# Picsart-AI-Research/StreamingT2V

Hardware: NVIDIA H100
Metric: denoise_steps_per_sec (higher is better)
Workload: dtype bf16

## Files before the change

streamingt2v_b200/csrc/mtgemm.cu:

```cuda
#include <cuda.h>
#include <cuda_bf16.h>
#include <stdlib.h>
#include <string.h>

#include "../../include/b200svd.h"
#include "common.h"
#include "mtgemm_ring.h"
#include "ptx.cuh"
#include "wgmma.cuh"

namespace b200 {

struct GemmDev {
  int32_t tap_off[B200SVD_MAX_TAPS][5];
  uint32_t taps, kblocks;
  uint32_t n;
  uint32_t n_tiles;
  uint32_t total_tiles;
  uint32_t m_ext[3];
  uint32_t m_lb[3];
  uint32_t m_tiles[3];
  uint32_t m_adim[3];
  int64_t out_rs[3];
  void* out;
  int64_t ldo;
  int32_t out_fp32;
  const float* bias;
  const float* fvec;
  int64_t ldf;
  uint32_t rows_per_frame;
  int32_t act;
  float s_acc;
  const __nv_bfloat16* res1;
  int64_t ld1;
  float s1;
  const __nv_bfloat16* res2;
  int64_t ld2;
  float s2;
  float* gn_part;
  int32_t* gn_slot_sample;
  int64_t gn_ld;
  uint32_t gn_rows;
  int32_t staged;
  int32_t epi_kind;
  uint32_t stages;
  uint32_t res_slots;
  uint32_t wg_off[3];
  const float* slope;
#ifdef MTGEMM_PHASE_CLOCKS
  long long* phase_buf;
// ... 69 lines not shown
  static constexpr int PRODUCER_REGS = 40;
  static constexpr int RES_SLOTS_AT_MIN = (SMEM_LIMIT - FIXED_BYTES - MIN_STAGES * STAGE_BYTES) / RES_SLOT_BYTES;
  static int res_slots_fit(int stages) { return (SMEM_LIMIT - FIXED_BYTES - stages * STAGE_BYTES) / RES_SLOT_BYTES; }
  static_assert(STAGES >= 4, "pipeline depth without residuals");
  static_assert(RES_SLOTS_AT_MIN >= 2, "two residuals need two ring slots");
  static_assert(STAGES * STAGE_BYTES + FIXED_BYTES <= SMEM_LIMIT, "shared memory budget");
  static_assert(STAGE_BYTES % 1024 == 0, "stage alignment");
  static_assert(BN % SUB_W == 0, "sub-tiles");
};

constexpr int ALT_STG_SLOT_BYTES = BM * SUB_W * 2;
constexpr int ALT_STG_BYTES = 2 * STG_SLOTS * ALT_STG_SLOT_BYTES;
template <int BN>
struct AltCfg {
  static constexpr int B_STAGE_BYTES = BN * BK * 2;
  static constexpr int STAGE_BYTES = A_STAGE_BYTES + B_STAGE_BYTES;
  static constexpr int FIXED = ALT_STG_BYTES + BAR_BYTES;
  static constexpr int STAGES_FIT = (SMEM_LIMIT - FIXED) / STAGE_BYTES;
  static constexpr int STAGES = STAGES_FIT > MAX_STAGES ? MAX_STAGES : STAGES_FIT;
  static constexpr int SUBTILES = BN / SUB_W;
  static constexpr int CONSUMER_REGS = 232;
  static constexpr int PRODUCER_REGS = 40;
  static constexpr int RES_SLOTS_AT_MIN = (SMEM_LIMIT - FIXED - MIN_STAGES * STAGE_BYTES) / RES_SLOT_BYTES;
  static int res_slots_fit(int stages) { return (SMEM_LIMIT - FIXED - stages * STAGE_BYTES) / RES_SLOT_BYTES; }
  static_assert(BN <= 128, "128 x BN accumulator in one warpgroup's registers");
  static_assert(2 * 128 * CONSUMER_REGS + 128 * PRODUCER_REGS <= 65536, "register file");
  static_assert(STAGES >= 4, "pipeline depth without residuals");
  static_assert(RES_SLOTS_AT_MIN >= 2, "two residuals need two ring slots");
  static_assert(STAGES * STAGE_BYTES + FIXED <= SMEM_LIMIT, "shared memory budget");
  static_assert(STAGE_BYTES % 1024 == 0, "stage alignment");
  static_assert(BN % SUB_W == 0, "sub-tiles");
};

__device__ __forceinline__ void decode_tile(const GemmDev& p, uint32_t tile, uint32_t& n_tile, uint32_t& mb1,
                                            uint32_t& mb2, uint32_t& mb3) {
  n_tile = tile % p.n_tiles;
  uint32_t mt = tile / p.n_tiles;
  const uint32_t t1 = mt % p.m_tiles[0];
  mt /= p.m_tiles[0];
  const uint32_t t2 = mt % p.m_tiles[1];
  const uint32_t t3 = mt / p.m_tiles[1];
  mb1 = t1 << p.m_lb[0];
  mb2 = t2 << p.m_lb[1];
  mb3 = t3 << p.m_lb[2];
}

__device__ __forceinline__ float ldg_bf16(const __nv_bfloat16* p) { return __bfloat162float(p[0]); }

__device__ __forceinline__ void load_bf16_pair(const __nv_bfloat16* base, int64_t i, bool both, float& a, float& b) {
  if (both && (i & 1) == 0) {
    const uint32_t w = __ldg(reinterpret_cast<const unsigned int*>(base + i));
    a = bf16_lo(w);
    b = bf16_hi(w);
  } else {
    a = ldg_bf16(base + i);
    b = both ? ldg_bf16(base + i + 1) : 0.f;
  }
}

__device__ __forceinline__ float epi_act(int act, float s_acc, float v, float g) {
  if (act == B200SVD_ACT_SILU) {
    v = silu_fast(v);
  } else if (act == B200SVD_ACT_GELU) {
    v = gelu_fast(v);
  } else if (act == B200SVD_ACT_GEGLU) {
    v = __fmul_rn(v, gelu_fast(g));
  } else if (act == B200SVD_ACT_PRELU) {
    v = v > 0.f ? v : __fmul_rn(g, v);
  }
  return __fmul_rn(v, s_acc);
// ... 162 lines not shown
#pragma unroll
    for (int o = 4; o < 32; o <<= 1) {
      gs0 += __shfl_xor_sync(0xffffffffu, gs0, o);
      gs1 += __shfl_xor_sync(0xffffffffu, gs1, o);
      gq0 += __shfl_xor_sync(0xffffffffu, gq0, o);
      gq1 += __shfl_xor_sync(0xffffffffu, gq1, o);
    }
    if (sender && first_row) *reinterpret_cast<float4*>(gxb + 2 * (8 * jj + 2 * cq)) = make_float4(gs0, gq0, gs1, gq1);
    if (!sender) {
      acc[4 * j] = gs0;
      acc[4 * j + 1] = gq0;
      acc[4 * j + 2] = gs1;
      acc[4 * j + 3] = gq1;
    }
  }
}

__device__ __forceinline__ void gn_write_partials(const GemmDev& p, const EpiTile& t, const float* acc, int c,
                                                  uint32_t cq, const float* gxb, uint32_t slot) {
  float2* dst = reinterpret_cast<float2*>(p.gn_part) + (int64_t)slot * p.gn_ld;
#pragma unroll
  for (int jj = 0; jj < 4; ++jj) {
    const int j = 4 * c + jj;
    const uint32_t ocol = t.otile0 + (uint32_t)(8 * j) + 2 * cq;
    if (ocol < t.n_out) {
      const float4 o = *reinterpret_cast<const float4*>(gxb + 2 * (8 * jj + 2 * cq));
      dst[ocol] = make_float2(acc[4 * j] + o.x, acc[4 * j + 1] + o.y);
      if (ocol + 1 < t.n_out) dst[ocol + 1] = make_float2(acc[4 * j + 2] + o.z, acc[4 * j + 3] + o.w);
    }
  }
}

template <int BN>
__device__ __forceinline__ void produce_ab(const GemmDev& p, const CUtensorMap* tmA, const CUtensorMap* tmB,
                                           uint8_t* smem, uint64_t* full_bar, uint64_t* empty_bar) {
  constexpr int STAGE_BYTES = A_STAGE_BYTES + BN * BK * 2;
  PhaseClock pc;
  uint32_t st = 0, ph = 0;
  for (uint32_t tile = blockIdx.x; tile < p.total_tiles; tile += gridDim.x) {
    uint32_t n_tile, mb1, mb2, mb3;
    decode_tile(p, tile, n_tile, mb1, mb2, mb3);
    int base[5] = {0, 0, 0, 0, 0};
    base[p.m_adim[0]] += (int)mb1;
    base[p.m_adim[1]] += (int)mb2;
    base[p.m_adim[2]] += (int)mb3;
    const int n0 = (int)(n_tile * BN);
    for (uint32_t tap = 0; tap < p.taps; ++tap) {
      const int c0 = p.tap_off[tap][0];
      const int c1 = base[1] + p.tap_off[tap][1];
      const int c2 = base[2] + p.tap_off[tap][2];
      const int c3 = base[3] + p.tap_off[tap][3];
      const int c4 = base[4] + p.tap_off[tap][4];
#pragma unroll 1
      for (uint32_t kb = 0; kb < p.kblocks; ++kb) {
        pc.mark(PC_OTHER);
        mbar_wait_parked(&empty_bar[st], ph ^ 1);
        pc.mark(PC_RING_WAIT);
        uint8_t* sa = smem + st * STAGE_BYTES;
        mbar_expect_tx(&full_bar[st], STAGE_BYTES);
        tma_load_5d(sa, tmA, &full_bar[st], c0 + (int)(kb * BK), c1, c2, c3, c4);
        tma_load_3d(sa + A_STAGE_BYTES, tmB, &full_bar[st], (int)(kb * BK), n0, (int)tap);
        if (++st == p.stages) {
          st = 0;
          ph ^= 1;
        }
      }
    }
  }
  pc.write(PC_BUF(p), 0);
}

__device__ __forceinline__ void produce_residuals(const GemmDev& p, const CUtensorMap* tmR1, const CUtensorMap* tmR2,
                                                  uint8_t* res_smem, uint64_t* res_full, uint64_t* res_empty,
                                                  uint32_t tile_out_w, uint32_t n_out) {
  if (p.res1 != nullptr) prefetch_tmap(tmR1);
  if (p.res2 != nullptr) prefetch_tmap(tmR2);
  uint32_t slot = 0, ph = 0;
  for (uint32_t tile = blockIdx.x; tile < p.total_tiles; tile += gridDim.x) {
    uint32_t n_tile, mb1, mb2, mb3;
    decode_tile(p, tile, n_tile, mb1, mb2, mb3);
    const uint32_t otile0 = n_tile * tile_out_w;
    for (uint32_t c = 0; c < tile_out_w / SUB_W && otile0 + c * SUB_W < n_out; ++c) {
      for (int r = 0; r < 2; ++r) {
        if ((r == 0 ? p.res1 : p.res2) == nullptr) continue;
        mbar_wait_parked(&res_empty[slot], ph ^ 1);
        mbar_expect_tx(&res_full[slot], RES_SLOT_BYTES);
        tma_load_4d(res_smem + slot * RES_SLOT_BYTES, r == 0 ? tmR1 : tmR2, &res_full[slot],
                    (int)(otile0 + c * SUB_W), (int)mb1, (int)mb2, (int)mb3);
        if (++slot == p.res_slots) {
          slot = 0;
          ph ^= 1;
        }
      }
    }
  }
}

template <int BN, class E, int HALVES>
__device__ __forceinline__ void epilogue_staged(const GemmDev& p, const CUtensorMap* tmO, const EpiTile& t,
                                                float* const (&acc)[HALVES], const OutRow (&rows)[HALVES][2],
                                                uint8_t* stg_smem, const uint8_t* res_smem, uint64_t* res_full,
                                                uint64_t* res_empty, RingPos& rr, uint32_t& stg_it, uint32_t cw,
                                                uint32_t rbase, uint32_t cq, bool leader, float* gn_x, PhaseClock& pc) {
  constexpr uint32_t SLOT_BYTES = HALVES * STG_SLOT_BYTES;
  const uint8_t* res_rows = res_smem + (HALVES == 1 ? cw * STG_SLOT_BYTES : 0u);
  const uint32_t wl = rbase >> 4, rq = rbase & 7u;
#pragma unroll
  for (int c = 0; c < BN / SUB_W; ++c) {
    if (E::geglu(p) && c >= BN / SUB_W / 2) break;
    if (t.otile0 + (uint32_t)(c * SUB_W) >= t.n_out) break;
    uint8_t* stg = stg_smem + (cw * STG_SLOTS + (stg_it & 1)) * SLOT_BYTES;
    float bv[4][2], gbv[4][2];
    epi_load_bias<BN, E>(p, t, c, cq, bv, gbv);
    const uint8_t* r1s = res_rows;
    const uint8_t* r2s = res_rows;
    uint32_t r1slot = 0, r2slot = 0;
    pc.mark(PC_EPI);
    if (E::res1(p)) {
      r1slot = rr.idx;
      mbar_wait(&res_full[rr.idx], rr.phase);
      r1s = res_rows + rr.idx * RES_SLOT_BYTES;
      ring_step(rr, p.res_slots);
    }
    if (E::res2(p)) {
      r2slot = rr.idx;
      mbar_wait(&res_full[rr.idx], rr.phase);
      r2s = res_rows + rr.idx * RES_SLOT_BYTES;
      ring_step(rr, p.res_slots);
// ... 2 lines not shown
#pragma unroll
    for (int hh = 0; hh < HALVES; ++hh)
      epi_stage_half<BN, E>(p, t, acc[hh], c, rbase, cq, stg + hh * STG_SLOT_BYTES, r1s + hh * STG_SLOT_BYTES,
                            r2s + hh * STG_SLOT_BYTES, bv, gbv, rows[hh]);
    float* gxb = nullptr;
    if constexpr (HALVES == 1 && E::GENERIC) {
      gxb = gn_x + ((cw * 2 + (stg_it & 1)) * 2 + (wl >> 1)) * (SUB_W * 2);
      if (p.gn_part != nullptr) gn_sum_partials<BN>(t, acc[0], c, rbase, cq, stg, rows[0], gxb, wl & 1, rq == 0);
    }
    fence_proxy_async_smem();
    pc.mark(PC_EPI);
    if (leader) tma_store_wait_read0();
    named_bar_sync(5 + (int)cw, 128);
    pc.mark(PC_STORE_WAIT);
    if (leader) {
      if (E::res1(p)) mbar_arrive(&res_empty[r1slot]);
      if (E::res2(p)) mbar_arrive(&res_empty[r2slot]);
      const bool second = HALVES == 1 && cw != 0;
      tma_store_4d(tmO, stg, (int)(t.otile0 + c * SUB_W), (int)(t.mb1 + (second ? p.wg_off[0] : 0u)),
                   (int)(t.mb2 + (second ? p.wg_off[1] : 0u)), (int)(t.mb3 + (second ? p.wg_off[2] : 0u)));
      tma_store_commit();
    }
    if constexpr (HALVES == 1 && E::GENERIC) {
      if (p.gn_part != nullptr && (wl & 1) == 0 && rq == 0)
        gn_write_partials(p, t, acc[0], c, cq, gxb, t.mt * 4u + 2 * cw + (wl >> 1));
    }
    ++stg_it;
  }
}

template <int BN>
__global__ void __launch_bounds__(NUM_THREADS, 1)
mtgemm_kernel(const __grid_constant__ CUtensorMap tmA, const __grid_constant__ CUtensorMap tmB,
              const __grid_constant__ CUtensorMap tmO, const __grid_constant__ CUtensorMap tmR1,
              const __grid_constant__ CUtensorMap tmR2, const GemmDev p) {
  using Cfg = TileCfg<BN>;
  constexpr int R = BN / 2;
  extern __shared__ __align__(1024) uint8_t smem[];
  if ((smem_u32(smem) & 1023u) != 0) __trap();
  const uint32_t stages = p.stages, rslots = p.res_slots;
  uint8_t* res_smem = smem + stages * Cfg::STAGE_BYTES;
  uint8_t* stg_smem = res_smem + rslots * RES_SLOT_BYTES;
  float* gn_x = reinterpret_cast<float*>(stg_smem + STG_BYTES);
  uint64_t* full_bar = reinterpret_cast<uint64_t*>(stg_smem + STG_BYTES + GN_BYTES);
  uint64_t* empty_bar = full_bar + MAX_STAGES;
  uint64_t* res_full = empty_bar + MAX_STAGES;
  uint64_t* res_empty = res_full + MAX_RES_SLOTS;

  const int warp = threadIdx.x >> 5;
  const int lane = threadIdx.x & 31;
  const int wg = warp >> 2;
  const uint32_t iters_per_tile = p.taps * p.kblocks;
  const bool geglu = (p.act == B200SVD_ACT_GEGLU);
  const uint32_t n_out = geglu ? p.n / 2 : p.n;
  const uint32_t tile_out_w = geglu ? (uint32_t)BN / 2 : (uint32_t)BN;

  if (threadIdx.x == 0) {
    prefetch_tmap(&tmA);
    prefetch_tmap(&tmB);
    if (p.staged) prefetch_tmap(&tmO);
    for (uint32_t s = 0; s < stages; ++s) {
      mbar_init(&full_bar[s], 1);
      mbar_init(&empty_bar[s], 2);
    }
    for (uint32_t s = 0; s < rslots; ++s) {
      mbar_init(&res_full[s], 1);
      mbar_init(&res_empty[s], 2);
    }
    fence_barrier_init();
  }
  __syncthreads();

  if (wg == 0) {
    asm volatile("setmaxnreg.dec.sync.aligned.u32 %0;" ::"n"(Cfg::PRODUCER_REGS));
    if (threadIdx.x == 0) {
      produce_ab<BN>(p, &tmA, &tmB, smem, full_bar, empty_bar);
    } else if (threadIdx.x == 32 && rslots != 0) {
      produce_residuals(p, &tmR1, &tmR2, res_smem, res_full, res_empty, tile_out_w, n_out);
    }
    return;
  }
  asm volatile("setmaxnreg.inc.sync.aligned.u32 %0;" ::"n"(Cfg::CONSUMER_REGS));

  const int cw = wg - 1;
  const int wl = warp & 3;
  const int rq = lane >> 2, cq = lane & 3;
  const bool leader = (threadIdx.x & 127) == 0;
  const uint32_t rbase = (uint32_t)(16 * wl + rq);
  RingPos ab = {0, 0};
  RingPos rr = {0, 0};
  uint32_t stg_it = 0;
  float acc[R];
  PhaseClock pc;

  for (uint32_t tile = blockIdx.x; tile < p.total_tiles; tile += gridDim.x) {
    pc.mark(PC_EPI);
#pragma unroll
    for (int i = 0; i < R; ++i) acc[i] = 0.f;
    uint32_t prev = 0;
    for (uint32_t i = 0; i < iters_per_tile; ++i) {
      mbar_wait(&full_bar[ab.idx], ab.phase);
      pc.mark(PC_RING_WAIT);
      const uint32_t sa = smem_u32(smem + ab.idx * Cfg::STAGE_BYTES);
      const uint64_t adesc = smem_desc_k_sw128(sa + cw * (A_STAGE_BYTES / 2));
      const uint64_t bdesc = smem_desc_k_sw128(sa + A_STAGE_BYTES);
      wgmma_fence_regs(acc);
      wgmma_fence();
#pragma unroll
      for (int kk = 0; kk < BK / 16; ++kk)
        Wgmma<BN>::ss(acc, adesc + (uint64_t)(kk * 2), bdesc + (uint64_t)(kk * 2), 1u);
      wgmma_commit();
      wgmma_fence_regs(acc);
      wgmma_wait<1>();
      pc.mark(PC_MMA);
      if (i > 0 && leader) mbar_arrive(&empty_bar[prev]);
      prev = ab.idx;
      ring_step(ab, stages);
    }
    wgmma_wait<0>();
    pc.mark(PC_MMA);
    wgmma_fence_regs(acc);
    if (leader) mbar_arrive(&empty_bar[prev]);

    uint32_t n_tile, mb1, mb2, mb3;
    decode_tile(p, tile, n_tile, mb1, mb2, mb3);
    const EpiTile et = {n_tile * BN, n_tile * tile_out_w, n_out, mb1, mb2, mb3, tile / p.n_tiles};
    const OutRow rows[1][2] = {{out_row(p, et, 64 * cw + rbase), out_row(p, et, 64 * cw + rbase + 8)}};
    if (p.staged) {
      float* const accs[1] = {acc};
      switch (p.epi_kind) {
        case B200SVD_EPI_GENERIC:
          epilogue_staged<BN, EpiGeneric, 1>(p, &tmO, et, accs, rows, stg_smem, res_smem, res_full, res_empty, rr,
                                             stg_it, cw, rbase, cq, leader, gn_x, pc);
          break;
#define MTGEMM_CASE(ID, ACT, BIAS, FVEC, NRES)                                                                    \
  case ID:                                                                                                        \
    if constexpr (ACT != B200SVD_ACT_GEGLU || BN == 128 || BN == 256)                                             \
      epilogue_staged<BN, Epi<ACT, BIAS, FVEC, NRES>, 1>(p, &tmO, et, accs, rows, stg_smem, res_smem, res_full,   \
                                                         res_empty, rr, stg_it, cw, rbase, cq, leader, gn_x, pc); \
    break;
        MTGEMM_EPI_KINDS(MTGEMM_CASE)
#undef MTGEMM_CASE
      }
      if (p.gn_part != nullptr && (wl & 1) == 0 && lane == 0 && n_tile == 0) {
        const uint32_t slot = et.mt * 4u + (uint32_t)(2 * cw + (wl >> 1));
        p.gn_slot_sample[slot] = rows[0][0].valid ? (int32_t)((uint32_t)rows[0][0].row / p.gn_rows) : -1;
      }
      continue;
    }
    constexpr int NJ = BN / 8;
#pragma unroll
    for (int j = 0; j < NJ; ++j) {
      if (geglu && j >= NJ / 2) break;
      const uint32_t tcol = 8 * j + 2 * cq;
      const uint32_t ocol = et.otile0 + tcol;
      const bool in0 = ocol < n_out, in1 = ocol + 1 < n_out;
#pragma unroll
      for (int h = 0; h < 2; ++h) {
        float v0 = acc[4 * j + 2 * h], v1 = acc[4 * j + 2 * h + 1];
// ... 25 lines not shown
          float a, b;
          load_bf16_pair(p.res1, row * p.ld1 + ocol, in1, a, b);
          v0 = __fmaf_rn(p.s1, a, v0);
          v1 = __fmaf_rn(p.s1, b, v1);
        }
        if (p.res2 != nullptr) {
          float a, b;
          load_bf16_pair(p.res2, row * p.ld2 + ocol, in1, a, b);
          v0 = __fmaf_rn(p.s2, a, v0);
          v1 = __fmaf_rn(p.s2, b, v1);
        }
        if (p.out_fp32) {
          float* op = reinterpret_cast<float*>(p.out) + row * p.ldo + ocol;
          if (in1 && ((row * p.ldo + ocol) & 1) == 0) {
            *reinterpret_cast<float2*>(op) = make_float2(v0, v1);
          } else {
            op[0] = v0;
            if (in1) op[1] = v1;
          }
        } else {
          __nv_bfloat16* op = reinterpret_cast<__nv_bfloat16*>(p.out) + row * p.ldo + ocol;
          if (in1) {
            *reinterpret_cast<uint32_t*>(op) = pack_bf16x2(v0, v1);
          } else {
            op[0] = __float2bfloat16(v0);
          }
        }
      }
    }
  }
  pc.mark(PC_EPI);
  if (leader) pc.write(PC_BUF(p), 1 + cw);
  if (p.staged && leader) tma_store_wait_all();
}

template <int BN>
__global__ void __launch_bounds__(NUM_THREADS, 1)
mtgemm_alt_kernel(const __grid_constant__ CUtensorMap tmA, const __grid_constant__ CUtensorMap tmB,
                  const __grid_constant__ CUtensorMap tmO, const __grid_constant__ CUtensorMap tmR1,
                  const __grid_constant__ CUtensorMap tmR2, const GemmDev p) {
  using Cfg = AltCfg<BN>;
  constexpr int R = BN / 2;
  extern __shared__ __align__(1024) uint8_t smem[];
  if ((smem_u32(smem) & 1023u) != 0) __trap();
  const uint32_t stages = p.stages, rslots = p.res_slots;
  uint8_t* res_smem = smem + stages * Cfg::STAGE_BYTES;
  uint8_t* stg_smem = res_smem + rslots * RES_SLOT_BYTES;
  uint64_t* full_bar = reinterpret_cast<uint64_t*>(stg_smem + ALT_STG_BYTES);
  uint64_t* empty_bar = full_bar + MAX_STAGES;
  uint64_t* res_full = empty_bar + MAX_STAGES;
  uint64_t* res_empty = res_full + MAX_RES_SLOTS;
  uint32_t* tiles_done = reinterpret_cast<uint32_t*>(res_empty + MAX_RES_SLOTS);

  const int warp = threadIdx.x >> 5;
  const int lane = threadIdx.x & 31;
  const int wg = warp >> 2;
  const uint32_t iters_per_tile = p.taps * p.kblocks;
  const bool geglu = (p.act == B200SVD_ACT_GEGLU);
  const uint32_t n_out = geglu ? p.n / 2 : p.n;
  const uint32_t tile_out_w = geglu ? (uint32_t)BN / 2 : (uint32_t)BN;

  if (threadIdx.x == 0) {
    prefetch_tmap(&tmA);
    prefetch_tmap(&tmB);
    prefetch_tmap(&tmO);
    for (int i = 0; i < 4; ++i) tiles_done[i] = 0;
    for (uint32_t s = 0; s < stages; ++s) {
      mbar_init(&full_bar[s], 1);
      mbar_init(&empty_bar[s], 1);
    }
    for (uint32_t s = 0; s < rslots; ++s) {
      mbar_init(&res_full[s], 1);
      mbar_init(&res_empty[s], 1);
    }
    fence_barrier_init();
  }
  __syncthreads();

  if (wg == 0) {
    asm volatile("setmaxnreg.dec.sync.aligned.u32 %0;" ::"n"(Cfg::PRODUCER_REGS));
    if (threadIdx.x == 0) {
      produce_ab<BN>(p, &tmA, &tmB, smem, full_bar, empty_bar);
    } else if (threadIdx.x == 32 && rslots != 0) {
      produce_residuals(p, &tmR1, &tmR2, res_smem, res_full, res_empty, tile_out_w, n_out);
    }
    return;
  }
  asm volatile("setmaxnreg.inc.sync.aligned.u32 %0;" ::"n"(Cfg::CONSUMER_REGS));

  const uint32_t cw = (uint32_t)(wg - 1);
  const int wl = warp & 3;
  const int rq = lane >> 2, cq = lane & 3;
  const bool leader = (threadIdx.x & 127) == 0;
  const uint32_t rbase = (uint32_t)(16 * wl + rq);
  const uint32_t nres = (p.res1 != nullptr ? 1u : 0u) + (p.res2 != nullptr ? 1u : 0u);
  RingPos ab = {0, 0};
  RingPos rr = {0, 0};
  uint32_t stg_it = 0;
  float acc0[R], acc1[R];
  PhaseClock pc;

  uint32_t t = 0;
  for (uint32_t tile = blockIdx.x; tile < p.total_tiles; tile += gridDim.x, ++t) {
    pc.mark(PC_EPI);
    if (alt_owner(t) != cw) {
      if (tile + gridDim.x >= p.total_tiles) break;
      ring_advance(ab, iters_per_tile, stages);
      if (rslots != 0) ring_advance(rr, tile_res_slots(tile % p.n_tiles, tile_out_w, n_out, SUB_W, nres), rslots);
      continue;
    }
    while (ld_acquire_shared(&tiles_done[1 - cw]) < t) {
    }
    pc.mark(PC_OTHER);
#pragma unroll
    for (int i = 0; i < R; ++i) acc0[i] = acc1[i] = 0.f;
    uint32_t prev = 0;
    for (uint32_t i = 0; i < iters_per_tile; ++i) {
      mbar_wait(&full_bar[ab.idx], ab.phase);
      pc.mark(PC_RING_WAIT);
      if (leader && i + 1 == iters_per_tile) st_release_shared(&tiles_done[cw], t + 1);
      const uint32_t sa = smem_u32(smem + ab.idx * Cfg::STAGE_BYTES);
      const uint64_t adesc0 = smem_desc_k_sw128(sa);
      const uint64_t adesc1 = smem_desc_k_sw128(sa + A_STAGE_BYTES / 2);
      const uint64_t bdesc = smem_desc_k_sw128(sa + A_STAGE_BYTES);
      wgmma_fence_regs(acc0);
      wgmma_fence_regs(acc1);
      wgmma_fence();
#pragma unroll
      for (int kk = 0; kk < BK / 16; ++kk) {
        Wgmma<BN>::ss(acc0, adesc0 + (uint64_t)(kk * 2), bdesc + (uint64_t)(kk * 2), 1u);
        Wgmma<BN>::ss(acc1, adesc1 + (uint64_t)(kk * 2), bdesc + (uint64_t)(kk * 2), 1u);
      }
      wgmma_commit();
      wgmma_fence_regs(acc0);
      wgmma_fence_regs(acc1);
      wgmma_wait<1>();
      pc.mark(PC_MMA);
      if (i > 0 && leader) mbar_arrive(&empty_bar[prev]);
      prev = ab.idx;
      ring_step(ab, stages);
    }
    wgmma_wait<0>();
    pc.mark(PC_MMA);
    wgmma_fence_regs(acc0);
    wgmma_fence_regs(acc1);
    if (leader) mbar_arrive(&empty_bar[prev]);

    uint32_t n_tile, mb1, mb2, mb3;
    decode_tile(p, tile, n_tile, mb1, mb2, mb3);
    const EpiTile et = {n_tile * BN, n_tile * tile_out_w, n_out, mb1, mb2, mb3, tile / p.n_tiles};
    const OutRow rows[2][2] = {{out_row(p, et, rbase), out_row(p, et, rbase + 8)},
                               {out_row(p, et, 64 + rbase), out_row(p, et, 64 + rbase + 8)}};
    if (rslots != 0) {
      pc.mark(PC_EPI);
      while (ld_acquire_shared(&tiles_done[2 + 1 - cw]) < t) {
      }
      pc.mark(PC_RES_WAIT);
    }
    float* const accs[2] = {acc0, acc1};
    switch (p.epi_kind) {
      case B200SVD_EPI_GENERIC:
        epilogue_staged<BN, EpiGeneric, 2>(p, &tmO, et, accs, rows, stg_smem, res_smem, res_full, res_empty, rr,
                                           stg_it, cw, rbase, cq, leader, nullptr, pc);
        break;
#define MTGEMM_CASE(ID, ACT, BIAS, FVEC, NRES)                                                                    \
  case ID:                                                                                                        \
    if constexpr (ACT != B200SVD_ACT_GEGLU || BN == 128)                                                          \
      epilogue_staged<BN, Epi<ACT, BIAS, FVEC, NRES>, 2>(p, &tmO, et, accs, rows, stg_smem, res_smem, res_full,   \
                                                         res_empty, rr, stg_it, cw, rbase, cq, leader, nullptr,   \
                                                         pc);                                                     \
    break;
      MTGEMM_EPI_KINDS(MTGEMM_CASE)
#undef MTGEMM_CASE
    }
    if (leader && rslots != 0) st_release_shared(&tiles_done[2 + cw], t + 1);
  }
  pc.mark(PC_EPI);
  if (leader) pc.write(PC_BUF(p), 1 + (int)cw);
  if (leader) tma_store_wait_all();
}

static int ilog2_exact(uint32_t v) {
  if (v == 0 || (v & (v - 1)) != 0) return -1;
  int l = 0;
  while ((1u << l) < v) ++l;
  return l;
}

struct EpiMaps {
  CUtensorMap out, res1, res2;
};

#ifdef MTGEMM_PHASE_CLOCKS
static long long* g_phase_buf = nullptr;
#endif

template <int BN, bool ALT>
struct SchedCfg {
  using type = TileCfg<BN>;
  static constexpr auto kernel = mtgemm_kernel<BN>;
};
template <int BN>
struct SchedCfg<BN, true> {
  using type = AltCfg<BN>;
  static constexpr auto kernel = mtgemm_alt_kernel<BN>;
};

template <int BN, bool ALT = false>
static int launch(const b200svd_gemm_params* p, const CUtensorMap& tmA, const EpiMaps& em, const GemmDev& d,
                  cudaStream_t st) {
  using Cfg = typename SchedCfg<BN, ALT>::type;
  constexpr auto kernel = SchedCfg<BN, ALT>::kernel;
  CUtensorMap tmB;
  uint64_t bd[3] = {p->k, p->n, p->taps};
  uint64_t bs[2] = {(uint64_t)p->k * 2, (uint64_t)p->k * 2 * p->n};
  uint32_t bb[3] = {64, (uint32_t)BN, 1};
  if (encode_tmap_bf16(&tmB, p->w_ptr, 3, bd, bs, bb)) return 1;
  GemmDev dd = d;
#ifdef MTGEMM_PHASE_CLOCKS
  dd.phase_buf = g_phase_buf;
#endif
  dd.n_tiles = (p->n + BN - 1) / BN;
  int stages = Cfg::STAGES, res_slots = 0;
  const int nres = d.staged ? (p->res1 != nullptr) + (p->res2 != nullptr) : 0;
  if (nres > 0) {
    const int tile_out_w = p->act == B200SVD_ACT_GEGLU ? BN / 2 : BN;
    int want = nres * (tile_out_w / SUB_W);
    if (want > MAX_RES_SLOTS) want = MAX_RES_SLOTS;
    while (stages > MIN_STAGES && Cfg::res_slots_fit(stages) < want) --stages;
    res_slots = Cfg::res_slots_fit(stages);
    if (res_slots > want) res_slots = want;
  }
  dd.stages = (uint32_t)stages;
  dd.res_slots = (uint32_t)res_slots;
  const int smem_bytes = stages * Cfg::STAGE_BYTES + res_slots * RES_SLOT_BYTES + Cfg::FIXED;
  const int slot = dev_slot();
  static bool attr_set[B200_MAX_DEVICES] = {};
  if (!attr_set[slot]) {
    cudaError_t e = cudaFuncSetAttribute(kernel, cudaFuncAttributeMaxDynamicSharedMemorySize, SMEM_LIMIT);
    if (e != cudaSuccess) return cuda_fail(e, "cudaFuncSetAttribute(mtgemm)");
    attr_set[slot] = true;
  }
  const uint64_t m_tiles = (uint64_t)dd.m_tiles[0] * dd.m_tiles[1] * dd.m_tiles[2];
  const uint64_t total = (uint64_t)dd.n_tiles * m_tiles;
  if (total == 0 || total > 0x7FFFFFFFull) {
    set_error("mtgemm: bad tile count %llu", (unsigned long long)total);
    return 1;
  }
  dd.total_tiles = (uint32_t)total;
  const uint32_t grid = (uint32_t)(total < (uint64_t)sm_count() ? total : (uint64_t)sm_count());
  kernel<<<grid, NUM_THREADS, smem_bytes, st>>>(tmA, tmB, em.out, em.res1, em.res2, dd);
  B200_CHECK_LAUNCH("mtgemm launch");
  return 0;
}

static int g_pair_mode = 2;

static int g_schedule = 2;
constexpr uint64_t ALT_MAX_TILE_MMA_CLOCKS = 20000;

static int alt_tile(int bn, bool geglu) {
  if (bn == 256 && !geglu) return 128;
  return bn <= 128 ? bn : 0;
}

static int g_epilogue = 1;

static int epilogue_kind(const b200svd_gemm_params* p) {
  const uint32_t n_out = p->act == B200SVD_ACT_GEGLU ? p->n / 2 : p->n;
  if (p->out_fp32 || n_out % 8 != 0 || p->gn_part != nullptr) return B200SVD_EPI_GENERIC;
  const bool bias = p->bias != nullptr, fvec = p->fvec != nullptr;
  const int nres = p->res1 == nullptr ? (p->res2 == nullptr ? 0 : -1) : (p->res2 == nullptr ? 1 : 2);
  if (!bias) return p->act == B200SVD_ACT_NONE && !fvec && nres == 0 ? B200SVD_EPI_PLAIN : B200SVD_EPI_GENERIC;
  switch (p->act) {
    case B200SVD_ACT_NONE:
      if (nres == 0) return fvec ? B200SVD_EPI_BIAS_FVEC : B200SVD_EPI_BIAS;
      if (nres == 1) return fvec ? B200SVD_EPI_BIAS_RES1_FVEC : B200SVD_EPI_BIAS_RES1;
      return nres == 2 && !fvec ? B200SVD_EPI_BIAS_RES2 : B200SVD_EPI_GENERIC;
    case B200SVD_ACT_SILU: return !fvec && nres == 0 ? B200SVD_EPI_BIAS_SILU : B200SVD_EPI_GENERIC;
    case B200SVD_ACT_GELU: return !fvec && nres == 0 ? B200SVD_EPI_BIAS_GELU : B200SVD_EPI_GENERIC;
    case B200SVD_ACT_GEGLU: return !fvec && nres == 0 ? B200SVD_EPI_BIAS_GEGLU : B200SVD_EPI_GENERIC;
    default: return B200SVD_EPI_GENERIC;
  }
}

}

extern "C" int b200svd_gemm_epilogue(int mode) {
  const int prev = b200::g_epilogue;
// ... 212 lines not shown
```

streamingt2v_b200/csrc/mtgemm_ring.h:

```cpp
#pragma once
#include <stdint.h>

#if defined(__CUDACC__)
#define MTGEMM_RING_FN __host__ __device__ __forceinline__
#else
#define MTGEMM_RING_FN inline
#endif

namespace b200 {

struct RingPos {
  uint32_t idx, phase;
};

MTGEMM_RING_FN void ring_step(RingPos& r, uint32_t depth) {
  if (++r.idx == depth) {
    r.idx = 0;
    r.phase ^= 1u;
  }
}

MTGEMM_RING_FN void ring_advance(RingPos& r, uint32_t n, uint32_t depth) {
  const uint32_t t = r.idx + n;
  r.phase ^= (t / depth) & 1u;
  r.idx = t % depth;
}

MTGEMM_RING_FN uint32_t alt_owner(uint32_t t) { return t & 1u; }

MTGEMM_RING_FN uint32_t tile_res_slots(uint32_t n_tile, uint32_t tile_out_w, uint32_t n_out, uint32_t sub_w,
                                       uint32_t nres) {
  const uint32_t o0 = n_tile * tile_out_w;
  if (o0 >= n_out) return 0;
  uint32_t c = (n_out - o0 + sub_w - 1) / sub_w;
  if (c > tile_out_w / sub_w) c = tile_out_w / sub_w;
  return c * nres;
}

}
```

streamingt2v_b200/csrc/ptx.cuh:

```cuda
#pragma once
#include <cuda.h>
#include <cuda_bf16.h>
#include <cuda_runtime.h>
#include <stdint.h>

namespace b200 {

__device__ __forceinline__ uint32_t smem_u32(const void* p) {
  return static_cast<uint32_t>(__cvta_generic_to_shared(p));
}

__device__ __forceinline__ void mbar_init(uint64_t* bar, uint32_t count) {
  asm volatile("mbarrier.init.shared::cta.b64 [%0], %1;" ::"r"(smem_u32(bar)), "r"(count));
}
__device__ __forceinline__ void fence_barrier_init() {
  asm volatile("fence.mbarrier_init.release.cluster;" ::: "memory");
}
__device__ __forceinline__ void fence_proxy_async_smem() {
  asm volatile("fence.proxy.async.shared::cta;" ::: "memory");
}
__device__ __forceinline__ void mbar_expect_tx(uint64_t* bar, uint32_t bytes) {
  asm volatile("mbarrier.arrive.expect_tx.shared::cta.b64 _, [%0], %1;" ::"r"(smem_u32(bar)), "r"(bytes)
               : "memory");
}
// ... 29 lines not shown

__device__ __forceinline__ void prefetch_tmap(const CUtensorMap* m) {
  asm volatile("prefetch.tensormap [%0];" ::"l"(reinterpret_cast<uint64_t>(m)) : "memory");
}
__device__ __forceinline__ void tma_load_2d(void* smem, const CUtensorMap* m, uint64_t* bar, int c0, int c1) {
  asm volatile(
      "cp.async.bulk.tensor.2d.shared::cluster.global.tile.mbarrier::complete_tx::bytes [%0], [%1, {%3, %4}], [%2];"
      ::"r"(smem_u32(smem)), "l"(reinterpret_cast<uint64_t>(m)), "r"(smem_u32(bar)), "r"(c0), "r"(c1)
      : "memory");
}
__device__ __forceinline__ void tma_load_3d(void* smem, const CUtensorMap* m, uint64_t* bar, int c0, int c1,
                                            int c2) {
  asm volatile(
      "cp.async.bulk.tensor.3d.shared::cluster.global.tile.mbarrier::complete_tx::bytes [%0], [%1, {%3, %4, %5}], "
      "[%2];" ::"r"(smem_u32(smem)),
      "l"(reinterpret_cast<uint64_t>(m)), "r"(smem_u32(bar)), "r"(c0), "r"(c1), "r"(c2)
      : "memory");
}
__device__ __forceinline__ void tma_load_4d(void* smem, const CUtensorMap* m, uint64_t* bar, int c0, int c1, int c2,
                                            int c3) {
  asm volatile(
      "cp.async.bulk.tensor.4d.shared::cluster.global.tile.mbarrier::complete_tx::bytes [%0], [%1, {%3, %4, %5, "
      "%6}], [%2];" ::"r"(smem_u32(smem)),
      "l"(reinterpret_cast<uint64_t>(m)), "r"(smem_u32(bar)), "r"(c0), "r"(c1), "r"(c2), "r"(c3)
      : "memory");
}
__device__ __forceinline__ void tma_load_5d(void* smem, const CUtensorMap* m, uint64_t* bar, int c0, int c1, int c2,
                                            int c3, int c4) {
  asm volatile(
      "cp.async.bulk.tensor.5d.shared::cluster.global.tile.mbarrier::complete_tx::bytes [%0], [%1, {%3, %4, %5, "
      "%6, %7}], [%2];" ::"r"(smem_u32(smem)),
      "l"(reinterpret_cast<uint64_t>(m)), "r"(smem_u32(bar)), "r"(c0), "r"(c1), "r"(c2), "r"(c3), "r"(c4)
      : "memory");
}

__device__ __forceinline__ void tma_store_4d(const CUtensorMap* m, const void* smem, int c0, int c1, int c2, int c3) {
  asm volatile(
      "cp.async.bulk.tensor.4d.global.shared::cta.tile.bulk_group [%0, {%2, %3, %4, %5}], [%1];" ::"l"(
          reinterpret_cast<uint64_t>(m)),
      "r"(smem_u32(smem)), "r"(c0), "r"(c1), "r"(c2), "r"(c3)
      : "memory");
}
__device__ __forceinline__ void tma_store_5d(const CUtensorMap* m, const void* smem, int c0, int c1, int c2, int c3,
                                             int c4) {
  asm volatile(
      "cp.async.bulk.tensor.5d.global.shared::cta.tile.bulk_group [%0, {%2, %3, %4, %5, %6}], [%1];" ::"l"(
          reinterpret_cast<uint64_t>(m)),
      "r"(smem_u32(smem)), "r"(c0), "r"(c1), "r"(c2), "r"(c3), "r"(c4)
      : "memory");
}
__device__ __forceinline__ void tma_store_commit() { asm volatile("cp.async.bulk.commit_group;" ::: "memory"); }
__device__ __forceinline__ void tma_store_wait_read0() { asm volatile("cp.async.bulk.wait_group.read 0;" ::: "memory"); }
template <int N>
__device__ __forceinline__ void tma_store_wait_read() {
  asm volatile("cp.async.bulk.wait_group.read %0;" ::"n"(N) : "memory");
}
__device__ __forceinline__ void tma_store_wait_all() { asm volatile("cp.async.bulk.wait_group 0;" ::: "memory"); }
__device__ __forceinline__ void named_bar_sync(int id, int nthreads) {
  asm volatile("bar.sync %0, %1;" ::"r"(id), "r"(nthreads) : "memory");
}

__device__ __forceinline__ void st_release_shared(uint32_t* p, uint32_t v) {
  asm volatile("st.release.cta.shared::cta.u32 [%0], %1;" ::"r"(smem_u32(p)), "r"(v) : "memory");
}
__device__ __forceinline__ uint32_t ld_acquire_shared(const uint32_t* p) {
  uint32_t v;
// ... 75 lines not shown
```

Measured before the change: 2.557.

## Pair CTAs into 2-CTA clusters that multicast shared weight tiles

Groups CTAs into clusters of two that process adjacent M tiles with the same N tile. Each CTA loads half of the weight (B) tile and multicasts it to both CTAs. Empty barriers now count arrivals from both CTAs, and phantom tiles fill odd M counts. This halves per-CTA weight traffic from L2/HBM, at the cost of cross-CTA synchronisation and possibly fewer resident clusters. By default (pair mode 2) it applies only to GEGLU GEMMs.

Measured after the change: 2.570, median of 6. No clear change (+0.5%).

```diff
diff --git a/streamingt2v_b200/csrc/mtgemm.cu b/streamingt2v_b200/csrc/mtgemm.cu
--- a/streamingt2v_b200/csrc/mtgemm.cu
+++ b/streamingt2v_b200/csrc/mtgemm.cu
@@ -16,6 +16,9 @@
   uint32_t taps, kblocks;
   uint32_t n;
   uint32_t n_tiles;
+  uint32_t m_tiles_all;
+  uint32_t csize;
+  uint32_t nclusters;
   uint32_t total_tiles;
   uint32_t m_ext[3];
   uint32_t m_lb[3];
@@ -151,10 +154,14 @@
   static_assert(BN % SUB_W == 0, "sub-tiles");
 };
 
-__device__ __forceinline__ void decode_tile(const GemmDev& p, uint32_t tile, uint32_t& n_tile, uint32_t& mb1,
-                                            uint32_t& mb2, uint32_t& mb3) {
-  n_tile = tile % p.n_tiles;
-  uint32_t mt = tile / p.n_tiles;
+__device__ __forceinline__ uint32_t cta_rank(const GemmDev& p) { return blockIdx.x & (p.csize - 1); }
+
+__device__ __forceinline__ ClusterTile cta_tile(const GemmDev& p, uint32_t ct) {
+  return cluster_tile(ct, p.n_tiles, p.m_tiles_all, p.csize, cta_rank(p));
+}
+
+__device__ __forceinline__ void decode_tile(const GemmDev& p, uint32_t mt, uint32_t& mb1, uint32_t& mb2,
+                                            uint32_t& mb3) {
   const uint32_t t1 = mt % p.m_tiles[0];
   mt /= p.m_tiles[0];
   const uint32_t t2 = mt % p.m_tiles[1];
@@ -383,19 +390,24 @@
 }
 
 template <int BN>
-__device__ __forceinline__ void produce_ab(const GemmDev& p, const CUtensorMap* tmA, const CUtensorMap* tmB,
-                                           uint8_t* smem, uint64_t* full_bar, uint64_t* empty_bar) {
-  constexpr int STAGE_BYTES = A_STAGE_BYTES + BN * BK * 2;
+__device__ __forceinline__ void produce_ab(const GemmDev& p, const CUtensorMap* tmA,
+                                           const CUtensorMap* tmB, const CUtensorMap* tmBh, uint8_t* smem,
+                                           uint64_t* full_bar, uint64_t* empty_bar) {
+  constexpr int B_STAGE_BYTES = BN * BK * 2;
+  constexpr int STAGE_BYTES = A_STAGE_BYTES + B_STAGE_BYTES;
+  static_assert((BN / 2) % 8 == 0, "a half weight box is whole 1024-byte swizzle atoms");
+  const uint32_t rank = cta_rank(p);
   PhaseClock pc;
   uint32_t st = 0, ph = 0;
-  for (uint32_t tile = blockIdx.x; tile < p.total_tiles; tile += gridDim.x) {
-    uint32_t n_tile, mb1, mb2, mb3;
-    decode_tile(p, tile, n_tile, mb1, mb2, mb3);
+  for (uint32_t ct = blockIdx.x / p.csize; ct < p.total_tiles; ct += p.nclusters) {
+    const ClusterTile t = cta_tile(p, ct);
+    uint32_t mb1, mb2, mb3;
+    decode_tile(p, t.m_tile, mb1, mb2, mb3);
     int base[5] = {0, 0, 0, 0, 0};
     base[p.m_adim[0]] += (int)mb1;
     base[p.m_adim[1]] += (int)mb2;
     base[p.m_adim[2]] += (int)mb3;
-    const int n0 = (int)(n_tile * BN);
+    const int n0 = (int)(t.n_tile * BN);
     for (uint32_t tap = 0; tap < p.taps; ++tap) {
       const int c0 = p.tap_off[tap][0];
       const int c1 = base[1] + p.tap_off[tap][1];
@@ -408,9 +420,14 @@
         mbar_wait_parked(&empty_bar[st], ph ^ 1);
         pc.mark(PC_RING_WAIT);
         uint8_t* sa = smem + st * STAGE_BYTES;
-        mbar_expect_tx(&full_bar[st], STAGE_BYTES);
-        tma_load_5d(sa, tmA, &full_bar[st], c0 + (int)(kb * BK), c1, c2, c3, c4);
-        tma_load_3d(sa + A_STAGE_BYTES, tmB, &full_bar[st], (int)(kb * BK), n0, (int)tap);
+        mbar_expect_tx(&full_bar[st], t.phantom ? B_STAGE_BYTES : STAGE_BYTES);
+        if (!t.phantom) tma_load_5d(sa, tmA, &full_bar[st], c0 + (int)(kb * BK), c1, c2, c3, c4);
+        if (p.csize == 1) {
+          tma_load_3d(sa + A_STAGE_BYTES, tmB, &full_bar[st], (int)(kb * BK), n0, (int)tap);
+        } else {
+          tma_load_3d_multicast(sa + A_STAGE_BYTES + rank * (B_STAGE_BYTES / 2), tmBh, &full_bar[st], 0x3,
+                                (int)(kb * BK), n0 + (int)rank * (BN / 2), (int)tap);
+        }
         if (++st == p.stages) {
           st = 0;
           ph ^= 1;
@@ -421,16 +438,18 @@
   pc.write(PC_BUF(p), 0);
 }
 
-__device__ __forceinline__ void produce_residuals(const GemmDev& p, const CUtensorMap* tmR1, const CUtensorMap* tmR2,
-                                                  uint8_t* res_smem, uint64_t* res_full, uint64_t* res_empty,
-                                                  uint32_t tile_out_w, uint32_t n_out) {
+__device__ __forceinline__ void produce_residuals(const GemmDev& p, const CUtensorMap* tmR1,
+                                                  const CUtensorMap* tmR2, uint8_t* res_smem, uint64_t* res_full,
+                                                  uint64_t* res_empty, uint32_t tile_out_w, uint32_t n_out) {
   if (p.res1 != nullptr) prefetch_tmap(tmR1);
   if (p.res2 != nullptr) prefetch_tmap(tmR2);
   uint32_t slot = 0, ph = 0;
-  for (uint32_t tile = blockIdx.x; tile < p.total_tiles; tile += gridDim.x) {
-    uint32_t n_tile, mb1, mb2, mb3;
-    decode_tile(p, tile, n_tile, mb1, mb2, mb3);
-    const uint32_t otile0 = n_tile * tile_out_w;
+  for (uint32_t ct = blockIdx.x / p.csize; ct < p.total_tiles; ct += p.nclusters) {
+    const ClusterTile t = cta_tile(p, ct);
+    if (t.phantom) continue;
+    uint32_t mb1, mb2, mb3;
+    decode_tile(p, t.m_tile, mb1, mb2, mb3);
+    const uint32_t otile0 = t.n_tile * tile_out_w;
     for (uint32_t c = 0; c < tile_out_w / SUB_W && otile0 + c * SUB_W < n_out; ++c) {
       for (int r = 0; r < 2; ++r) {
         if ((r == 0 ? p.res1 : p.res2) == nullptr) continue;
@@ -445,6 +464,11 @@
       }
     }
   }
+}
+
+__device__ __forceinline__ void release_stage(const GemmDev& p, uint64_t* bar) {
+  mbar_arrive(bar);
+  if (p.csize == 2) mbar_arrive_remote(bar, cta_rank(p) ^ 1u);
 }
 
 template <int BN, class E, int HALVES>
@@ -513,8 +537,8 @@
 template <int BN>
 __global__ void __launch_bounds__(NUM_THREADS, 1)
 mtgemm_kernel(const __grid_constant__ CUtensorMap tmA, const __grid_constant__ CUtensorMap tmB,
-              const __grid_constant__ CUtensorMap tmO, const __grid_constant__ CUtensorMap tmR1,
-              const __grid_constant__ CUtensorMap tmR2, const GemmDev p) {
+              const __grid_constant__ CUtensorMap tmBh, const __grid_constant__ CUtensorMap tmO,
+              const __grid_constant__ CUtensorMap tmR1, const __grid_constant__ CUtensorMap tmR2, const GemmDev p) {
   using Cfg = TileCfg<BN>;
   constexpr int R = BN / 2;
   extern __shared__ __align__(1024) uint8_t smem[];
@@ -535,14 +559,13 @@
   const bool geglu = (p.act == B200SVD_ACT_GEGLU);
   const uint32_t n_out = geglu ? p.n / 2 : p.n;
   const uint32_t tile_out_w = geglu ? (uint32_t)BN / 2 : (uint32_t)BN;
-
   if (threadIdx.x == 0) {
     prefetch_tmap(&tmA);
-    prefetch_tmap(&tmB);
+    prefetch_tmap(p.csize == 1 ? &tmB : &tmBh);
     if (p.staged) prefetch_tmap(&tmO);
     for (uint32_t s = 0; s < stages; ++s) {
       mbar_init(&full_bar[s], 1);
-      mbar_init(&empty_bar[s], 2);
+      mbar_init(&empty_bar[s], 2 * p.csize);
     }
     for (uint32_t s = 0; s < rslots; ++s) {
       mbar_init(&res_full[s], 1);
@@ -550,15 +573,20 @@
     }
     fence_barrier_init();
   }
-  __syncthreads();
+  if (p.csize > 1) {
+    cluster_sync();
+  } else {
+    __syncthreads();
+  }
 
   if (wg == 0) {
     asm volatile("setmaxnreg.dec.sync.aligned.u32 %0;" ::"n"(Cfg::PRODUCER_REGS));
     if (threadIdx.x == 0) {
-      produce_ab<BN>(p, &tmA, &tmB, smem, full_bar, empty_bar);
+      produce_ab<BN>(p, &tmA, &tmB, &tmBh, smem, full_bar, empty_bar);
     } else if (threadIdx.x == 32 && rslots != 0) {
       produce_residuals(p, &tmR1, &tmR2, res_smem, res_full, res_empty, tile_out_w, n_out);
     }
+    if (p.csize > 1) cluster_sync();
     return;
   }
   asm volatile("setmaxnreg.inc.sync.aligned.u32 %0;" ::"n"(Cfg::CONSUMER_REGS));
@@ -574,7 +602,8 @@
   float acc[R];
   PhaseClock pc;
 
-  for (uint32_t tile = blockIdx.x; tile < p.total_tiles; tile += gridDim.x) {
+  for (uint32_t ct = blockIdx.x / p.csize; ct < p.total_tiles; ct += p.nclusters) {
+    const bool phantom = cta_tile(p, ct).phantom;
     pc.mark(PC_EPI);
 #pragma unroll
     for (int i = 0; i < R; ++i) acc[i] = 0.f;
@@ -582,30 +611,35 @@
     for (uint32_t i = 0; i < iters_per_tile; ++i) {
       mbar_wait(&full_bar[ab.idx], ab.phase);
       pc.mark(PC_RING_WAIT);
-      const uint32_t sa = smem_u32(smem + ab.idx * Cfg::STAGE_BYTES);
-      const uint64_t adesc = smem_desc_k_sw128(sa + cw * (A_STAGE_BYTES / 2));
-      const uint64_t bdesc = smem_desc_k_sw128(sa + A_STAGE_BYTES);
-      wgmma_fence_regs(acc);
-      wgmma_fence();
-#pragma unroll
-      for (int kk = 0; kk < BK / 16; ++kk)
-        Wgmma<BN>::ss(acc, adesc + (uint64_t)(kk * 2), bdesc + (uint64_t)(kk * 2), 1u);
-      wgmma_commit();
-      wgmma_fence_regs(acc);
+      if (!phantom) {
+        const uint32_t sa = smem_u32(smem + ab.idx * Cfg::STAGE_BYTES);
+        const uint64_t adesc = smem_desc_k_sw128(sa + cw * (A_STAGE_BYTES / 2));
+        const uint64_t bdesc = smem_desc_k_sw128(sa + A_STAGE_BYTES);
+        wgmma_fence_regs(acc);
+        wgmma_fence();
+#pragma unroll
+        for (int kk = 0; kk < BK / 16; ++kk)
+          Wgmma<BN>::ss(acc, adesc + (uint64_t)(kk * 2), bdesc + (uint64_t)(kk * 2), 1u);
+        wgmma_commit();
+        wgmma_fence_regs(acc);
+      }
       wgmma_wait<1>();
       pc.mark(PC_MMA);
-      if (i > 0 && leader) mbar_arrive(&empty_bar[prev]);
+      if (i > 0 && leader) release_stage(p, &empty_bar[prev]);
       prev = ab.idx;
       ring_step(ab, stages);
     }
     wgmma_wait<0>();
     pc.mark(PC_MMA);
     wgmma_fence_regs(acc);
-    if (leader) mbar_arrive(&empty_bar[prev]);
-
-    uint32_t n_tile, mb1, mb2, mb3;
-    decode_tile(p, tile, n_tile, mb1, mb2, mb3);
-    const EpiTile et = {n_tile * BN, n_tile * tile_out_w, n_out, mb1, mb2, mb3, tile / p.n_tiles};
+    if (leader) release_stage(p, &empty_bar[prev]);
+    if (phantom) continue;
+
+    const ClusterTile ctl = cta_tile(p, ct);
+    const uint32_t n_tile = ctl.n_tile;
+    uint32_t mb1, mb2, mb3;
+    decode_tile(p, ctl.m_tile, mb1, mb2, mb3);
+    const EpiTile et = {n_tile * BN, n_tile * tile_out_w, n_out, mb1, mb2, mb3, ctl.m_tile};
     const OutRow rows[1][2] = {{out_row(p, et, 64 * cw + rbase), out_row(p, et, 64 * cw + rbase + 8)}};
     if (p.staged) {
       float* const accs[1] = {acc};
@@ -697,13 +731,15 @@
   pc.mark(PC_EPI);
   if (leader) pc.write(PC_BUF(p), 1 + cw);
   if (p.staged && leader) tma_store_wait_all();
+  if (p.csize > 1) cluster_sync();
 }
 
 template <int BN>
 __global__ void __launch_bounds__(NUM_THREADS, 1)
 mtgemm_alt_kernel(const __grid_constant__ CUtensorMap tmA, const __grid_constant__ CUtensorMap tmB,
-                  const __grid_constant__ CUtensorMap tmO, const __grid_constant__ CUtensorMap tmR1,
-                  const __grid_constant__ CUtensorMap tmR2, const GemmDev p) {
+                  const __grid_constant__ CUtensorMap tmBh, const __grid_constant__ CUtensorMap tmO,
+                  const __grid_constant__ CUtensorMap tmR1, const __grid_constant__ CUtensorMap tmR2,
+                  const GemmDev p) {
   using Cfg = AltCfg<BN>;
   constexpr int R = BN / 2;
   extern __shared__ __align__(1024) uint8_t smem[];
@@ -724,15 +760,14 @@
   const bool geglu = (p.act == B200SVD_ACT_GEGLU);
   const uint32_t n_out = geglu ? p.n / 2 : p.n;
   const uint32_t tile_out_w = geglu ? (uint32_t)BN / 2 : (uint32_t)BN;
-
   if (threadIdx.x == 0) {
     prefetch_tmap(&tmA);
-    prefetch_tmap(&tmB);
+    prefetch_tmap(p.csize == 1 ? &tmB : &tmBh);
     prefetch_tmap(&tmO);
     for (int i = 0; i < 4; ++i) tiles_done[i] = 0;
     for (uint32_t s = 0; s < stages; ++s) {
       mbar_init(&full_bar[s], 1);
-      mbar_init(&empty_bar[s], 1);
+      mbar_init(&empty_bar[s], p.csize);
     }
     for (uint32_t s = 0; s < rslots; ++s) {
       mbar_init(&res_full[s], 1);
@@ -740,15 +775,20 @@
     }
     fence_barrier_init();
   }
-  __syncthreads();
+  if (p.csize > 1) {
+    cluster_sync();
+  } else {
+    __syncthreads();
+  }
 
   if (wg == 0) {
     asm volatile("setmaxnreg.dec.sync.aligned.u32 %0;" ::"n"(Cfg::PRODUCER_REGS));
     if (threadIdx.x == 0) {
-      produce_ab<BN>(p, &tmA, &tmB, smem, full_bar, empty_bar);
+      produce_ab<BN>(p, &tmA, &tmB, &tmBh, smem, full_bar, empty_bar);
     } else if (threadIdx.x == 32 && rslots != 0) {
       produce_residuals(p, &tmR1, &tmR2, res_smem, res_full, res_empty, tile_out_w, n_out);
     }
+    if (p.csize > 1) cluster_sync();
     return;
   }
   asm volatile("setmaxnreg.inc.sync.aligned.u32 %0;" ::"n"(Cfg::CONSUMER_REGS));
@@ -766,14 +806,16 @@
   PhaseClock pc;
 
   uint32_t t = 0;
-  for (uint32_t tile = blockIdx.x; tile < p.total_tiles; tile += gridDim.x, ++t) {
+  for (uint32_t ct = blockIdx.x / p.csize; ct < p.total_tiles; ct += p.nclusters, ++t) {
     pc.mark(PC_EPI);
     if (alt_owner(t) != cw) {
-      if (tile + gridDim.x >= p.total_tiles) break;
+      if (ct + p.nclusters >= p.total_tiles) break;
       ring_advance(ab, iters_per_tile, stages);
-      if (rslots != 0) ring_advance(rr, tile_res_slots(tile % p.n_tiles, tile_out_w, n_out, SUB_W, nres), rslots);
+      if (rslots != 0)
+        ring_advance(rr, cta_tile_res_slots(cta_tile(p, ct), tile_out_w, n_out, SUB_W, nres), rslots);
       continue;
     }
+    const bool phantom = cta_tile(p, ct).phantom;
     while (ld_acquire_shared(&tiles_done[1 - cw]) < t) {
     }
     pc.mark(PC_OTHER);
@@ -784,24 +826,26 @@
       mbar_wait(&full_bar[ab.idx], ab.phase);
       pc.mark(PC_RING_WAIT);
       if (leader && i + 1 == iters_per_tile) st_release_shared(&tiles_done[cw], t + 1);
-      const uint32_t sa = smem_u32(smem + ab.idx * Cfg::STAGE_BYTES);
-      const uint64_t adesc0 = smem_desc_k_sw128(sa);
-      const uint64_t adesc1 = smem_desc_k_sw128(sa + A_STAGE_BYTES / 2);
-      const uint64_t bdesc = smem_desc_k_sw128(sa + A_STAGE_BYTES);
-      wgmma_fence_regs(acc0);
-      wgmma_fence_regs(acc1);
-      wgmma_fence();
-#pragma unroll
-      for (int kk = 0; kk < BK / 16; ++kk) {
-        Wgmma<BN>::ss(acc0, adesc0 + (uint64_t)(kk * 2), bdesc + (uint64_t)(kk * 2), 1u);
-        Wgmma<BN>::ss(acc1, adesc1 + (uint64_t)(kk * 2), bdesc + (uint64_t)(kk * 2), 1u);
-      }
-      wgmma_commit();
-      wgmma_fence_regs(acc0);
-      wgmma_fence_regs(acc1);
+      if (!phantom) {
+        const uint32_t sa = smem_u32(smem + ab.idx * Cfg::STAGE_BYTES);
+        const uint64_t adesc0 = smem_desc_k_sw128(sa);
+        const uint64_t adesc1 = smem_desc_k_sw128(sa + A_STAGE_BYTES / 2);
+        const uint64_t bdesc = smem_desc_k_sw128(sa + A_STAGE_BYTES);
+        wgmma_fence_regs(acc0);
+        wgmma_fence_regs(acc1);
+        wgmma_fence();
+#pragma unroll
+        for (int kk = 0; kk < BK / 16; ++kk) {
+          Wgmma<BN>::ss(acc0, adesc0 + (uint64_t)(kk * 2), bdesc + (uint64_t)(kk * 2), 1u);
+          Wgmma<BN>::ss(acc1, adesc1 + (uint64_t)(kk * 2), bdesc + (uint64_t)(kk * 2), 1u);
+        }
+        wgmma_commit();
+        wgmma_fence_regs(acc0);
+        wgmma_fence_regs(acc1);
+      }
       wgmma_wait<1>();
       pc.mark(PC_MMA);
-      if (i > 0 && leader) mbar_arrive(&empty_bar[prev]);
+      if (i > 0 && leader) release_stage(p, &empty_bar[prev]);
       prev = ab.idx;
       ring_step(ab, stages);
     }
@@ -809,19 +853,25 @@
     pc.mark(PC_MMA);
     wgmma_fence_regs(acc0);
     wgmma_fence_regs(acc1);
-    if (leader) mbar_arrive(&empty_bar[prev]);
-
-    uint32_t n_tile, mb1, mb2, mb3;
-    decode_tile(p, tile, n_tile, mb1, mb2, mb3);
-    const EpiTile et = {n_tile * BN, n_tile * tile_out_w, n_out, mb1, mb2, mb3, tile / p.n_tiles};
-    const OutRow rows[2][2] = {{out_row(p, et, rbase), out_row(p, et, rbase + 8)},
-                               {out_row(p, et, 64 + rbase), out_row(p, et, 64 + rbase + 8)}};
+    if (leader) release_stage(p, &empty_bar[prev]);
+
     if (rslots != 0) {
       pc.mark(PC_EPI);
       while (ld_acquire_shared(&tiles_done[2 + 1 - cw]) < t) {
       }
       pc.mark(PC_RES_WAIT);
     }
+    if (phantom) {
+      if (leader && rslots != 0) st_release_shared(&tiles_done[2 + cw], t + 1);
+      continue;
+    }
+    const ClusterTile ctl = cta_tile(p, ct);
+    const uint32_t n_tile = ctl.n_tile;
+    uint32_t mb1, mb2, mb3;
+    decode_tile(p, ctl.m_tile, mb1, mb2, mb3);
+    const EpiTile et = {n_tile * BN, n_tile * tile_out_w, n_out, mb1, mb2, mb3, ctl.m_tile};
+    const OutRow rows[2][2] = {{out_row(p, et, rbase), out_row(p, et, rbase + 8)},
+                               {out_row(p, et, 64 + rbase), out_row(p, et, 64 + rbase + 8)}};
     float* const accs[2] = {acc0, acc1};
     switch (p.epi_kind) {
       case B200SVD_EPI_GENERIC:
@@ -843,6 +893,7 @@
   pc.mark(PC_EPI);
   if (leader) pc.write(PC_BUF(p), 1 + (int)cw);
   if (leader) tma_store_wait_all();
+  if (p.csize > 1) cluster_sync();
 }
 
 static int ilog2_exact(uint32_t v) {
@@ -871,16 +922,18 @@
   static constexpr auto kernel = mtgemm_alt_kernel<BN>;
 };
 
+static int g_pair_mode = 2;
+
+static bool use_pairs(uint64_t m_tiles, int pair_clusters, bool geglu) {
+  if (m_tiles < 2 || pair_clusters < 1) return false;
+  return g_pair_mode == 1 || g_pair_mode == 3 || (g_pair_mode == 2 && geglu);
+}
+
 template <int BN, bool ALT = false>
 static int launch(const b200svd_gemm_params* p, const CUtensorMap& tmA, const EpiMaps& em, const GemmDev& d,
                   cudaStream_t st) {
   using Cfg = typename SchedCfg<BN, ALT>::type;
   constexpr auto kernel = SchedCfg<BN, ALT>::kernel;
-  CUtensorMap tmB;
-  uint64_t bd[3] = {p->k, p->n, p->taps};
-  uint64_t bs[2] = {(uint64_t)p->k * 2, (uint64_t)p->k * 2 * p->n};
-  uint32_t bb[3] = {64, (uint32_t)BN, 1};
-  if (encode_tmap_bf16(&tmB, p->w_ptr, 3, bd, bs, bb)) return 1;
   GemmDev dd = d;
 #ifdef MTGEMM_PHASE_CLOCKS
   dd.phase_buf = g_phase_buf;
@@ -901,9 +954,23 @@
   const int smem_bytes = stages * Cfg::STAGE_BYTES + res_slots * RES_SLOT_BYTES + Cfg::FIXED;
   const int slot = dev_slot();
   static bool attr_set[B200_MAX_DEVICES] = {};
+  static int pair_clusters[B200_MAX_DEVICES] = {};
+  cudaLaunchAttribute cluster;
+  cluster.id = cudaLaunchAttributeClusterDimension;
+  cluster.val.clusterDim.y = cluster.val.clusterDim.z = 1;
+  cudaLaunchConfig_t cfg = {};
+  cfg.blockDim = dim3(NUM_THREADS);
+  cfg.stream = st;
   if (!attr_set[slot]) {
     cudaError_t e = cudaFuncSetAttribute(kernel, cudaFuncAttributeMaxDynamicSharedMemorySize, SMEM_LIMIT);
     if (e != cudaSuccess) return cuda_fail(e, "cudaFuncSetAttribute(mtgemm)");
+    cluster.val.clusterDim.x = 2;
+    cfg.gridDim = dim3(2 * (uint32_t)((sm_count() + 1) / 2));
+    cfg.dynamicSmemBytes = SMEM_LIMIT;
+    cfg.attrs = &cluster;
+    cfg.numAttrs = 1;
+    e = cudaOccupancyMaxActiveClusters(&pair_clusters[slot], kernel, &cfg);
+    if (e != cudaSuccess) return cuda_fail(e, "cudaOccupancyMaxActiveClusters(mtgemm)");
     attr_set[slot] = true;
   }
   const uint64_t m_tiles = (uint64_t)dd.m_tiles[0] * dd.m_tiles[1] * dd.m_tiles[2];
@@ -912,14 +979,32 @@
     set_error("mtgemm: bad tile count %llu", (unsigned long long)total);
     return 1;
   }
-  dd.total_tiles = (uint32_t)total;
-  const uint32_t grid = (uint32_t)(total < (uint64_t)sm_count() ? total : (uint64_t)sm_count());
-  kernel<<<grid, NUM_THREADS, smem_bytes, st>>>(tmA, tmB, em.out, em.res1, em.res2, dd);
-  B200_CHECK_LAUNCH("mtgemm launch");
+  const uint32_t cs = use_pairs(m_tiles, pair_clusters[slot], p->act == B200SVD_ACT_GEGLU) ? 2 : 1;
+  dd.m_tiles_all = (uint32_t)m_tiles;
+  dd.csize = cs;
+  dd.total_tiles = cluster_tile_count(dd.n_tiles, dd.m_tiles_all, cs);
+  const uint32_t max_clusters = cs == 1 ? (uint32_t)sm_count() : (uint32_t)pair_clusters[slot];
+  const uint32_t clusters = dd.total_tiles < max_clusters ? dd.total_tiles : max_clusters;
+  dd.nclusters = clusters;
+  CUtensorMap tmB, tmBh;
+  uint64_t bd[3] = {p->k, p->n, p->taps};
+  uint64_t bs[2] = {(uint64_t)p->k * 2, (uint64_t)p->k * 2 * p->n};
+  uint32_t bb[3] = {64, (uint32_t)BN, 1};
+  if (encode_tmap_bf16(&tmB, p->w_ptr, 3, bd, bs, bb)) return 1;
+  tmBh = tmB;
+  if (cs == 2) {
+    bb[1] = BN / 2;
+    if (encode_tmap_bf16(&tmBh, p->w_ptr, 3, bd, bs, bb)) return 1;
+  }
+  cluster.val.clusterDim.x = cs;
+  cfg.gridDim = dim3(clusters * cs);
+  cfg.dynamicSmemBytes = (size_t)smem_bytes;
+  cfg.attrs = &cluster;
+  cfg.numAttrs = cs == 1 ? 0 : 1;
+  const cudaError_t e = cudaLaunchKernelEx(&cfg, kernel, tmA, tmB, tmBh, em.out, em.res1, em.res2, dd);
+  if (e != cudaSuccess) return cuda_fail(e, "mtgemm launch");
   return 0;
 }
-
-static int g_pair_mode = 2;
 
 static int g_schedule = 2;
 constexpr uint64_t ALT_MAX_TILE_MMA_CLOCKS = 20000;
diff --git a/streamingt2v_b200/csrc/mtgemm_ring.h b/streamingt2v_b200/csrc/mtgemm_ring.h
--- a/streamingt2v_b200/csrc/mtgemm_ring.h
+++ b/streamingt2v_b200/csrc/mtgemm_ring.h
@@ -37,4 +37,27 @@
   return c * nres;
 }
 
+struct ClusterTile {
+  uint32_t n_tile, m_tile;
+  bool phantom;
+};
+
+MTGEMM_RING_FN uint32_t cluster_tile_count(uint32_t n_tiles, uint32_t m_tiles, uint32_t csize) {
+  return n_tiles * ((m_tiles + csize - 1) / csize);
 }
+
+MTGEMM_RING_FN ClusterTile cluster_tile(uint32_t ct, uint32_t n_tiles, uint32_t m_tiles, uint32_t csize,
+                                        uint32_t rank) {
+  ClusterTile t;
+  t.n_tile = ct % n_tiles;
+  t.m_tile = ct / n_tiles * csize + rank;
+  t.phantom = t.m_tile >= m_tiles;
+  return t;
+}
+
+MTGEMM_RING_FN uint32_t cta_tile_res_slots(const ClusterTile& t, uint32_t tile_out_w, uint32_t n_out, uint32_t sub_w,
+                                           uint32_t nres) {
+  return t.phantom ? 0u : tile_res_slots(t.n_tile, tile_out_w, n_out, sub_w, nres);
+}
+
+}
diff --git a/streamingt2v_b200/csrc/ptx.cuh b/streamingt2v_b200/csrc/ptx.cuh
--- a/streamingt2v_b200/csrc/ptx.cuh
+++ b/streamingt2v_b200/csrc/ptx.cuh
@@ -85,6 +85,27 @@
       "%6, %7}], [%2];" ::"r"(smem_u32(smem)),
       "l"(reinterpret_cast<uint64_t>(m)), "r"(smem_u32(bar)), "r"(c0), "r"(c1), "r"(c2), "r"(c3), "r"(c4)
       : "memory");
+}
+
+__device__ __forceinline__ void tma_load_3d_multicast(void* smem, const CUtensorMap* m, uint64_t* bar,
+                                                      uint16_t cta_mask, int c0, int c1, int c2) {
+  asm volatile(
+      "cp.async.bulk.tensor.3d.shared::cluster.global.tile.mbarrier::complete_tx::bytes.multicast::cluster [%0], [%1, "
+      "{%4, %5, %6}], [%2], %3;" ::"r"(smem_u32(smem)),
+      "l"(reinterpret_cast<uint64_t>(m)), "r"(smem_u32(bar)), "h"(cta_mask), "r"(c0), "r"(c1), "r"(c2)
+      : "memory");
+}
+
+__device__ __forceinline__ void mbar_arrive_remote(uint64_t* bar, uint32_t cta) {
+  asm volatile(
+      "{\n\t.reg .b32 ra;\n\t"
+      "mapa.shared::cluster.u32 ra, %0, %1;\n\t"
+      "mbarrier.arrive.shared::cluster.b64 _, [ra];\n\t}" ::"r"(smem_u32(bar)),
+      "r"(cta)
+      : "memory");
+}
+__device__ __forceinline__ void cluster_sync() {
+  asm volatile("barrier.cluster.arrive.release;\n\tbarrier.cluster.wait.acquire;" ::: "memory");
 }
 
 __device__ __forceinline__ void tma_store_4d(const CUtensorMap* m, const void* smem, int c0, int c1, int c2, int c3) {
```
